# rskew/aiko_services

Measured on AMD Instinct MI355X. Metric: frames/sec (whole node) + p50 latency, ResNet-50 pipeline at 1/2/4/8 MI355X, higher is better.
Workload: dtype bf16; 1 GPU; global_batch=640, per_gpu_batch=640, parallelism=dp1, hipgraph=True, ingest=hbm, setup_frames=12, model=resnet50, pipeline=(SyntheticFrames ResNet50Classifier ClassifierTopK), gpu_lanes=2

## Files before the change

aiko_services_amd/csrc/kernels/conv_exp.hip:

```cpp
#include <type_traits>

#include "conv_common.h"
#include "conv_wide_stage.h"

namespace aiko {

typedef __attribute__((ext_vector_type(2))) short i16x2;

__device__ __forceinline__ uint32_t relu_bf16x2(uint32_t v) {
  return __builtin_bit_cast(uint32_t, __builtin_elementwise_max(__builtin_bit_cast(i16x2, v), i16x2{0, 0}));
}

struct ConvExpParams {
  ConvParams c;
  const bf16_t* w3;
  const float* b3;
  int N;
};

__global__ __launch_bounds__(512, 1) void conv3x3_exp_kernel(ConvExpParams q) {
  const ConvParams& p = q.c;
  constexpr int BM = 256, BN = 256, BK = 64, WGN = 4, NW = 8, NS = 2;
  constexpr int WM = 128, WN = 64, MI = 8, NI = 4, NP = 2;
  constexpr int RPW = 8, RPI = 64, APT = 4, BPT = 4;
  constexpr int STAGE_ELEMS = (BM + BN) * BK;
  constexpr int T2_BLOCK = BM * 64;
  static_assert(NS * STAGE_ELEMS == 4 * T2_BLOCK, "the t2 slice fills the ring exactly");
  __shared__ __attribute__((aligned(16))) bf16_t ring[NS * STAGE_ELEMS];

  const int wave = __builtin_amdgcn_readfirstlane(threadIdx.x >> 6);
  const int wr = wave / WGN, wc = wave % WGN;
  const int ntiles = (p.M + BM - 1) / BM;
  const int G = gridDim.x;
  const int lid = xcd_remap(blockIdx.x, G);

  const __amdgpu_buffer_rsrc_t rx = wide_rsrc(p.x);
  const __amdgpu_buffer_rsrc_t rw = wide_rsrc(p.w);
  const __amdgpu_buffer_rsrc_t rw3 = wide_rsrc(q.w3);
  const int io_bytes = p.M * q.N * 2;
  const __amdgpu_buffer_rsrc_t rr =
      __builtin_amdgcn_make_buffer_rsrc(const_cast<bf16_t*>(p.res), (short)0, io_bytes, 0x00020000);
  const __amdgpu_buffer_rsrc_t ry = __builtin_amdgcn_make_buffer_rsrc(p.y, (short)0, io_bytes, 0x00020000);

  const int nkb = p.K / BK;
  const int nch = q.N / 128;

  for (int tile = lid; tile < ntiles; tile += G) {
    const int m0 = tile * BM;
    uint32_t lz = 0u;
    asm volatile("" : "+v"(lz));
    const int lane1 = __builtin_amdgcn_mbcnt_hi(~0u, __builtin_amdgcn_mbcnt_lo(~0u, lz));
    const int lrow = wave * RPW + (lane1 >> 3);
    const int lp = (lane1 & 7) ^ (lane1 >> 3);
    const int HoWo = p.Ho * p.Wo;
    uint32_t b_off[BPT];
#pragma unroll
    for (int i = 0; i < BPT; ++i) b_off[i] = (uint32_t)(((lrow + RPI * i) * p.K + lp * 8) * 2);

    const int fr = lane1 & 15, fq = lane1 >> 4;
    const int coff = ((fq & 1) << 4) | ((fq >> 1) << 3);
    const int sw = fr & 7;

    int a_base[APT];
    uint32_t a_mask[APT], a_off[APT];
#pragma unroll
    for (int i = 0; i < APT; ++i) {
      const int m = m0 + lrow + RPI * i;
      a_mask[i] = 0u;
      a_base[i] = 0;
      a_off[i] = kWideOOB;
      if (m < p.M) {
        const int img = fdiv(m, p.mHoWo, p.lHoWo);
        const int rem = m - img * HoWo;
        const int oh = fdiv(rem, p.mWo, p.lWo);
        const int ow = rem - oh * p.Wo;
        const int ih0 = oh * p.stride - p.pad, iw0 = ow * p.stride - p.pad;
        a_base[i] = (((img * p.H + ih0) * p.W + iw0) * p.C + lp * 8) * 2;
        const int r_lo = max(0, -ih0), r_hi = min(p.R, p.H - ih0);
        const int s_lo = max(0, -iw0), s_hi = min(p.S, p.W - iw0);
        const uint32_t mr = r_hi > r_lo ? ((1u << r_hi) - 1u) & ~((1u << r_lo) - 1u) : 0u;
        const uint32_t ms = s_hi > s_lo ? ((1u << s_hi) - 1u) & ~((1u << s_lo) - 1u) : 0u;
        a_mask[i] = mr | (ms << 16);
      }
    }
    float e_bias[NP][8];
#pragma unroll
    for (int h = 0; h < NP; ++h) {
      const int n = wc * WN + h * 32 + coff;
      const f32x4 b0 = *reinterpret_cast<const f32x4*>(p.bias + n);
      const f32x4 b1 = *reinterpret_cast<const f32x4*>(p.bias + n + 4);
      e_bias[h][0] = b0[0]; e_bias[h][1] = b0[1]; e_bias[h][2] = b0[2]; e_bias[h][3] = b0[3];
      e_bias[h][4] = b1[0]; e_bias[h][5] = b1[1]; e_bias[h][6] = b1[2]; e_bias[h][7] = b1[3];
    }

    int cur_tap = -1, iss_tap = 0, iss_c = 0, iss_r = 0, iss_s = 0;
    auto issue = [&](int kb, auto slot_tag) {
      constexpr int SLOT = decltype(slot_tag)::value;
      bf16_t* Xs = ring + SLOT * STAGE_ELEMS;
      bf16_t* Ws = Xs + BM * BK;
      const uint32_t sb = (uint32_t)(kb * BK * 2);
#pragma unroll
      for (int i = 0; i < BPT; ++i) wide_dma16(rw, b_off[i], sb, Ws + (i * RPI + wave * RPW) * BK);
      if (iss_tap != cur_tap) {
        cur_tap = iss_tap;
        const int tap_off = ((iss_r * p.W + iss_s) * p.C) * 2;
        const uint32_t bit = (1u << iss_r) | (1u << (iss_s + 16));
#pragma unroll
        for (int i = 0; i < APT; ++i)
          a_off[i] = (a_mask[i] & bit) == bit ? (uint32_t)(a_base[i] + tap_off) : kWideOOB;
      }
      const uint32_t soff = (uint32_t)(iss_c * 2);
#pragma unroll
      for (int i = 0; i < APT; ++i) wide_dma16(rx, a_off[i], soff, Xs + (i * RPI + wave * RPW) * BK);
      iss_c += BK;
      if (iss_c >= p.Cc) {
        iss_c = 0;
        ++iss_tap;
        if (++iss_s == p.S) {
          iss_s = 0;
          ++iss_r;
        }
      }
    };

    f32x4 acc[NI][MI];
    float zero = 0.f;
    asm volatile("" : "+v"(zero));
#pragma unroll
    for (int j = 0; j < NI; ++j)
#pragma unroll
      for (int i = 0; i < MI; ++i) acc[j][i] = f32x4{zero, zero, zero, zero};

    int w_rd[NI], x_rd[MI];
#pragma unroll
    for (int j = 0; j < NI; ++j) w_rd[j] = BM * BK + (wc * WN + j * 16 + fr) * BK;
#pragma unroll
    for (int i = 0; i < MI; ++i) x_rd[i] = (wr * WM + i * 16 + fr) * BK;

    auto compute = [&](auto slot_tag) {
      constexpr int SLOT = decltype(slot_tag)::value;
      const bf16_t* St = ring + SLOT * STAGE_ELEMS;
#pragma unroll
      for (int kk = 0; kk < BK / 32; ++kk) {
        const int pc = ((fq + 4 * kk) ^ sw) << 3;
        bf16x8 wf[NI], xf[MI];
#pragma unroll
        for (int j = 0; j < NI; ++j) wf[j] = *reinterpret_cast<const bf16x8*>(St + w_rd[j] + pc);
#pragma unroll
        for (int i = 0; i < MI; ++i) xf[i] = *reinterpret_cast<const bf16x8*>(St + x_rd[i] + pc);
#pragma unroll
        for (int i = 0; i < MI; ++i)
#pragma unroll
          for (int j = 0; j < NI; ++j)
            acc[j][i] = __builtin_amdgcn_mfma_f32_16x16x32_bf16(wf[j], xf[i], acc[j][i], 0, 0, 0);
      }
    };

    auto step = [&](int kb, auto slot_tag) {
      constexpr int SLOT = decltype(slot_tag)::value;
      wide_vm_barrier<0>();
      if (kb + 1 < nkb) issue(kb + 1, std::integral_constant<int, 1 - SLOT>{});
      compute(slot_tag);
    };
    using S0 = std::integral_constant<int, 0>;
    using S1 = std::integral_constant<int, 1>;
    issue(0, S0{});
    {
      int kb = 0;
      for (; kb + 2 <= nkb; kb += 2) {
        step(kb, S0{});
        step(kb + 1, S1{});
      }
      if (kb < nkb) step(kb, S0{});
    }

    uint32_t lz2 = 0u;
    asm volatile("" : "+v"(lz2));
    const int lane2 = __builtin_amdgcn_mbcnt_hi(~0u, __builtin_amdgcn_mbcnt_lo(~0u, lz2));
    const int fr2 = lane2 & 15, fq2 = lane2 >> 4;
    const int coff2 = ((fq2 & 1) << 4) | ((fq2 >> 1) << 3);
    const int sw2 = fr2 & 7;
    const int x_r0 = (wr * WM + fr2) * 64;
    __syncthreads();
#pragma unroll
    for (int i = 0; i < MI; ++i) {
#pragma unroll
      for (int h = 0; h < NP; ++h) {
        f32x4 lo = acc[2 * h][i], hi = acc[2 * h + 1][i];
#pragma unroll
        for (int e = 0; e < 4; ++e) {
          const auto s = __builtin_amdgcn_permlane16_swap(__float_as_uint(lo[e]), __float_as_uint(hi[e]), false, false);
          lo[e] = __uint_as_float(s[0]);
          hi[e] = __uint_as_float(s[1]);
        }
        u32x4 o;
        o[0] = pack2(fmaxf(lo[0] + e_bias[h][0], 0.f), fmaxf(lo[1] + e_bias[h][1], 0.f));
        o[1] = pack2(fmaxf(lo[2] + e_bias[h][2], 0.f), fmaxf(lo[3] + e_bias[h][3], 0.f));
        o[2] = pack2(fmaxf(hi[0] + e_bias[h][4], 0.f), fmaxf(hi[1] + e_bias[h][5], 0.f));
        o[3] = pack2(fmaxf(hi[2] + e_bias[h][6], 0.f), fmaxf(hi[3] + e_bias[h][7], 0.f));
        const int piece = (h * 4 + (coff2 >> 3)) ^ sw2;
        *reinterpret_cast<u32x4*>(ring + wc * T2_BLOCK + (x_r0 + i * 16 * 64) + (piece << 3)) = o;
      }
    }

    const uint32_t row0 = (uint32_t)(((m0 + wr * WM + fr2) * q.N + wc * 32 + coff2) * 2);
    const uint32_t row_step = (uint32_t)(16 * q.N * 2);
    const uint32_t w_off = (uint32_t)(wc * 2 * 8 * 1024 + lane2 * 16);
    bf16x8 wreg[4][2];
    u32x4 e_res[2][MI];
    f32x2 e_b3[4];
    auto load_w = [&](int c, int ks) __attribute__((always_inline)) {
      const uint32_t base = c < nch ? w_off : kWideOOB;
#pragma unroll
      for (int j = 0; j < 2; ++j)
        wreg[ks & 3][j] = __builtin_bit_cast(bf16x8, __builtin_amdgcn_raw_buffer_load_b128(
            rw3, base, (uint32_t)c * 65536u + (uint32_t)((j * 8 + ks) * 1024), 0));
    };
    auto load_res = [&](int c, auto par_tag) __attribute__((always_inline)) {
      constexpr int P = decltype(par_tag)::value;
      const uint32_t cb = (uint32_t)c * 256u;
      const uint32_t base = c < nch ? row0 : kWideOOB;
      uint32_t rs = row_step;
      asm volatile("" : "+s"(rs));
#pragma unroll
      for (int i = 0; i < MI; ++i)
        e_res[P][i] = __builtin_bit_cast(u32x4, __builtin_amdgcn_raw_buffer_load_b128(
            rr, base + rs * i, cb, 0));
    };
    auto load_b3 = [&](int c) __attribute__((always_inline)) {
      const int n = c * 128 + wc * 32 + coff2;
      const f32x4 b0 = *reinterpret_cast<const f32x4*>(q.b3 + n);
      const f32x4 b1 = *reinterpret_cast<const f32x4*>(q.b3 + n + 4);
      e_b3[0] = f32x2{b0[0], b0[1]}; e_b3[1] = f32x2{b0[2], b0[3]};
      e_b3[2] = f32x2{b1[0], b1[1]}; e_b3[3] = f32x2{b1[2], b1[3]};
    };
    using P0 = std::integral_constant<int, 0>;
    using P1 = std::integral_constant<int, 1>;
#pragma unroll
    for (int ks = 0; ks < 4; ++ks) load_w(0, ks);
    load_res(0, P0{});
    load_res(1, P1{});
    __syncthreads();

    const bf16_t* xa[2][2];
#pragma unroll
    for (int par = 0; par < 2; ++par)
#pragma unroll
      for (int half = 0; half < 2; ++half)
        xa[par][half] = ring + half * 2 * T2_BLOCK + x_r0 + (((fq2 + 4 * par) ^ sw2) << 3);
    auto read_x = [&](int ks, int i) __attribute__((always_inline)) {
      return *reinterpret_cast<const bf16x8*>(xa[ks & 1][ks >> 2] + ((ks >> 1) & 1) * T2_BLOCK + i * 16 * 64);
    };
    bf16x8 xf[MI];
#pragma unroll
    for (int i = 0; i < MI; ++i) xf[i] = read_x(0, i);
    auto chunk = [&](int c, auto par_tag) __attribute__((always_inline)) {
      constexpr int P = decltype(par_tag)::value;
      asm volatile("" ::: "memory");
      f32x4 acc2[2][MI];
#pragma unroll
      for (int j = 0; j < 2; ++j)
#pragma unroll
        for (int i = 0; i < MI; ++i) acc2[j][i] = f32x4{0.f, 0.f, 0.f, 0.f};
      load_b3(c);
#pragma unroll
      for (int ks = 0; ks < 8; ++ks) {
#pragma unroll
        for (int i = 0; i < MI; ++i) {
#pragma unroll
          for (int j = 0; j < 2; ++j)
            acc2[j][i] = __builtin_amdgcn_mfma_f32_16x16x32_bf16(wreg[ks & 3][j], xf[i], acc2[j][i], 0, 0, 0);
          xf[i] = read_x((ks + 1) & 7, i);
          __builtin_amdgcn_sched_barrier(0);
        }
        if (ks < 4) load_w(c, ks + 4);
        else load_w(c + 1, ks - 4);
        __builtin_amdgcn_sched_barrier(0);
      }
      const uint32_t cb = (uint32_t)c * 256u;
      uint32_t rs = row_step;
      asm volatile("" : "+s"(rs));
#pragma unroll
      for (int i = 0; i < MI; ++i) {
        f32x4 lo = acc2[0][i], hi = acc2[1][i];
#pragma unroll
        for (int e = 0; e < 4; ++e) {
          const auto s = __builtin_amdgcn_permlane16_swap(__float_as_uint(lo[e]), __float_as_uint(hi[e]), false, false);
          lo[e] = __uint_as_float(s[0]);
          hi[e] = __uint_as_float(s[1]);
        }
        const f32x2 v[4] = {f32x2{lo[0], lo[1]} + e_b3[0], f32x2{lo[2], lo[3]} + e_b3[1],
                            f32x2{hi[0], hi[1]} + e_b3[2], f32x2{hi[2], hi[3]} + e_b3[3]};
        u32x4 o;
#pragma unroll
        for (int e = 0; e < 4; ++e) {
          const f32x2 r = {__uint_as_float(e_res[P][i][e] << 16), __uint_as_float(e_res[P][i][e] & 0xffff0000u)};
          const f32x2 t = v[e] + r;
          o[e] = relu_bf16x2(pack2(t[0], t[1]));
        }
        __builtin_amdgcn_raw_buffer_store_b128(o, ry, row0 + rs * i, cb, 0);
        asm volatile("s_nop 1");
        __builtin_amdgcn_sched_barrier(0);
      }
      load_res(c + 2, par_tag);
    };
    for (int c = 0; c < nch; c += 2) {
      chunk(c, P0{});
      chunk(c + 1, P1{});
    }
    __syncthreads();
  }
}

}

extern "C" int aiko_conv3x3_exp(const void* t1, const void* w2, const float* b2, const void* w3img,
                                const float* b3, const void* res, void* y, int B, int H, int W, int N,
                                int grid, hipStream_t stream) {
  using namespace aiko;
  const long M = (long)B * H * W;
  if (N <= 0 || N % 256 || M <= 0 || M * N * 2 >= 0x7ffffff0L || H * W <= 0 || grid < 0) return -1;
  ConvExpParams q;
  ConvParams& p = q.c;
  p.x = static_cast<const bf16_t*>(t1);
  p.w = static_cast<const bf16_t*>(w2);
  p.bias = b2;
  p.res = static_cast<const bf16_t*>(res);
  p.y = static_cast<bf16_t*>(y);
  p.H = H; p.W = W; p.C = 256; p.Cc = 256; p.R = 3; p.S = 3;
  p.stride = 1; p.pad = 1; p.Ho = H; p.Wo = W; p.M = (int)M; p.Cout = 256; p.K = 9 * 256;
  p.act = 1; p.ldy = N; p.ldr = N;
  p.x2 = nullptr;
  p.K1 = p.K; p.H2 = 0; p.W2 = 0; p.C2 = 0; p.stride2 = 1;
  conv_params_finalize(p);
  q.w3 = static_cast<const bf16_t*>(w3img);
  q.b3 = b3;
  q.N = N;
  const int ntiles = (int)((M + 255) / 256);
  const int g = grid > 0 && grid < ntiles ? grid : ntiles;
  conv3x3_exp_kernel<<<dim3(g), 512, 0, stream>>>(q);
  return (int)hipGetLastError();
}
```

Before: 100,000 frames/s.

## Stage expansion-conv weights through LDS with async DMA double buffering

Templates the fused 3x3+1x1 expansion kernel on a W3_LDS flag. When enabled (the default), the 1x1 weights for each chunk are DMA'd into two extra LDS slots ahead of use, with vmcnt waits and barriers between steps, instead of each wave loading them directly into registers. This aims to hide weight-load latency and cut redundant global traffic. In exchange it adds block-wide barriers per k-step and more LDS per block. An environment variable selects the old path.

```diff
diff --git a/aiko_services_amd/csrc/kernels/conv_exp.hip b/aiko_services_amd/csrc/kernels/conv_exp.hip
--- a/aiko_services_amd/csrc/kernels/conv_exp.hip
+++ b/aiko_services_amd/csrc/kernels/conv_exp.hip
@@ -1,3 +1,4 @@
+#include <cstdlib>
 #include <type_traits>
 
 #include "conv_common.h"
@@ -18,6 +19,7 @@
   int N;
 };
 
+template <bool W3_LDS>
 __global__ __launch_bounds__(512, 1) void conv3x3_exp_kernel(ConvExpParams q) {
   const ConvParams& p = q.c;
   constexpr int BM = 256, BN = 256, BK = 64, WGN = 4, NW = 8, NS = 2;
@@ -25,8 +27,10 @@
   constexpr int RPW = 8, RPI = 64, APT = 4, BPT = 4;
   constexpr int STAGE_ELEMS = (BM + BN) * BK;
   constexpr int T2_BLOCK = BM * 64;
+  constexpr int W3_SLOT = 128 * 64;
   static_assert(NS * STAGE_ELEMS == 4 * T2_BLOCK, "the t2 slice fills the ring exactly");
-  __shared__ __attribute__((aligned(16))) bf16_t ring[NS * STAGE_ELEMS];
+  static_assert((NS * STAGE_ELEMS + 2 * W3_SLOT) * 2 <= 160 * 1024, "LDS budget");
+  __shared__ __attribute__((aligned(16))) bf16_t ring[NS * STAGE_ELEMS + (W3_LDS ? 2 * W3_SLOT : 0)];
 
   const int wave = __builtin_amdgcn_readfirstlane(threadIdx.x >> 6);
   const int wr = wave / WGN, wc = wave % WGN;
@@ -181,7 +185,20 @@
     const int coff2 = ((fq2 & 1) << 4) | ((fq2 >> 1) << 3);
     const int sw2 = fr2 & 7;
     const int x_r0 = (wr * WM + fr2) * 64;
+    const int nst = nch * 4;
+    const uint32_t w_lane = (uint32_t)lane2 * 16u;
+    auto issue_w = [&](int g, int slot) __attribute__((always_inline)) {
+      bf16_t* dst = ring + NS * STAGE_ELEMS + slot * W3_SLOT + wave * 1024;
+      const uint32_t voff = g < nst ? w_lane : kWideOOB;
+      const uint32_t soff = (uint32_t)(g >> 2) * 65536u + (uint32_t)(wave * 8192 + (g & 3) * 2048);
+      wide_dma16(rw3, voff, soff, dst);
+      wide_dma16(rw3, voff, soff + 1024u, dst + 512);
+    };
     __syncthreads();
+    if constexpr (W3_LDS) {
+      issue_w(0, 0);
+      issue_w(1, 1);
+    }
 #pragma unroll
     for (int i = 0; i < MI; ++i) {
 #pragma unroll
@@ -236,11 +253,34 @@
     };
     using P0 = std::integral_constant<int, 0>;
     using P1 = std::integral_constant<int, 1>;
-#pragma unroll
-    for (int ks = 0; ks < 4; ++ks) load_w(0, ks);
-    load_res(0, P0{});
-    load_res(1, P1{});
-    __syncthreads();
+    auto epilogue = [&](int c, auto par_tag, f32x4 (&acc2)[2][MI]) __attribute__((always_inline)) {
+      constexpr int P = decltype(par_tag)::value;
+      const uint32_t cb = (uint32_t)c * 256u;
+      uint32_t rs = row_step;
+      asm volatile("" : "+s"(rs));
+#pragma unroll
+      for (int i = 0; i < MI; ++i) {
+        f32x4 lo = acc2[0][i], hi = acc2[1][i];
+#pragma unroll
+        for (int e = 0; e < 4; ++e) {
+          const auto s = __builtin_amdgcn_permlane16_swap(__float_as_uint(lo[e]), __float_as_uint(hi[e]), false, false);
+          lo[e] = __uint_as_float(s[0]);
+          hi[e] = __uint_as_float(s[1]);
+        }
+        const f32x2 v[4] = {f32x2{lo[0], lo[1]} + e_b3[0], f32x2{lo[2], lo[3]} + e_b3[1],
+                            f32x2{hi[0], hi[1]} + e_b3[2], f32x2{hi[2], hi[3]} + e_b3[3]};
+        u32x4 o;
+#pragma unroll
+        for (int e = 0; e < 4; ++e) {
+          const f32x2 r = {__uint_as_float(e_res[P][i][e] << 16), __uint_as_float(e_res[P][i][e] & 0xffff0000u)};
+          const f32x2 t = v[e] + r;
+          o[e] = relu_bf16x2(pack2(t[0], t[1]));
+        }
+        __builtin_amdgcn_raw_buffer_store_b128(o, ry, row0 + rs * i, cb, 0);
+        asm volatile("s_nop 1");
+        __builtin_amdgcn_sched_barrier(0);
+      }
+    };
 
     const bf16_t* xa[2][2];
 #pragma unroll
@@ -252,61 +292,104 @@
       return *reinterpret_cast<const bf16x8*>(xa[ks & 1][ks >> 2] + ((ks >> 1) & 1) * T2_BLOCK + i * 16 * 64);
     };
     bf16x8 xf[MI];
-#pragma unroll
-    for (int i = 0; i < MI; ++i) xf[i] = read_x(0, i);
-    auto chunk = [&](int c, auto par_tag) __attribute__((always_inline)) {
-      constexpr int P = decltype(par_tag)::value;
-      asm volatile("" ::: "memory");
-      f32x4 acc2[2][MI];
-#pragma unroll
-      for (int j = 0; j < 2; ++j)
-#pragma unroll
-        for (int i = 0; i < MI; ++i) acc2[j][i] = f32x4{0.f, 0.f, 0.f, 0.f};
-      load_b3(c);
-#pragma unroll
-      for (int ks = 0; ks < 8; ++ks) {
-#pragma unroll
-        for (int i = 0; i < MI; ++i) {
+    if constexpr (!W3_LDS) {
+#pragma unroll
+      for (int ks = 0; ks < 4; ++ks) load_w(0, ks);
+      load_res(0, P0{});
+      load_res(1, P1{});
+      __syncthreads();
+#pragma unroll
+      for (int i = 0; i < MI; ++i) xf[i] = read_x(0, i);
+      auto chunk = [&](int c, auto par_tag) __attribute__((always_inline)) {
+        asm volatile("" ::: "memory");
+        f32x4 acc2[2][MI];
+#pragma unroll
+        for (int j = 0; j < 2; ++j)
+#pragma unroll
+          for (int i = 0; i < MI; ++i) acc2[j][i] = f32x4{0.f, 0.f, 0.f, 0.f};
+        load_b3(c);
+#pragma unroll
+        for (int ks = 0; ks < 8; ++ks) {
+#pragma unroll
+          for (int i = 0; i < MI; ++i) {
+#pragma unroll
+            for (int j = 0; j < 2; ++j)
+              acc2[j][i] = __builtin_amdgcn_mfma_f32_16x16x32_bf16(wreg[ks & 3][j], xf[i], acc2[j][i], 0, 0, 0);
+            xf[i] = read_x((ks + 1) & 7, i);
+            __builtin_amdgcn_sched_barrier(0);
+          }
+          if (ks < 4) load_w(c, ks + 4);
+          else load_w(c + 1, ks - 4);
+          __builtin_amdgcn_sched_barrier(0);
+        }
+        epilogue(c, par_tag, acc2);
+        load_res(c + 2, par_tag);
+      };
+      for (int c = 0; c < nch; c += 2) {
+        chunk(c, P0{});
+        chunk(c + 1, P1{});
+      }
+    } else {
+      load_res(0, P0{});
+      wide_vm_barrier<10>();
+      const bf16_t* wrd = ring + NS * STAGE_ELEMS + wc * 2048 + lane2 * 8;
+      u32x4 wA[2][2], wB[2][2];
+      auto read_w = [&](auto slot_tag, u32x4 (&w)[2][2]) __attribute__((always_inline)) {
+        constexpr int SLOT = decltype(slot_tag)::value;
+#pragma unroll
+        for (int sl = 0; sl < 2; ++sl)
 #pragma unroll
           for (int j = 0; j < 2; ++j)
-            acc2[j][i] = __builtin_amdgcn_mfma_f32_16x16x32_bf16(wreg[ks & 3][j], xf[i], acc2[j][i], 0, 0, 0);
-          xf[i] = read_x((ks + 1) & 7, i);
-          __builtin_amdgcn_sched_barrier(0);
-        }
-        if (ks < 4) load_w(c, ks + 4);
-        else load_w(c + 1, ks - 4);
+            w[sl][j] = *reinterpret_cast<const u32x4*>(wrd + SLOT * W3_SLOT + j * 1024 + sl * 512);
+      };
+      auto step = [&](int c, auto kb_tag, auto par_tag, f32x4 (&acc2)[2][MI]) __attribute__((always_inline)) {
+        constexpr int KB = decltype(kb_tag)::value, CUR = KB & 1, P = decltype(par_tag)::value;
+        u32x4 (&wcur)[2][2] = CUR ? wB : wA;
+        u32x4 (&wnxt)[2][2] = CUR ? wA : wB;
+        asm volatile("s_waitcnt vmcnt(%4)\n\ts_barrier"
+                     : "+v"(wcur[0][0]), "+v"(wcur[0][1]), "+v"(wcur[1][0]), "+v"(wcur[1][1])
+                     : "n"(KB < 2 ? 8 : 0)
+                     : "memory");
+        issue_w(c * 4 + KB + 2, CUR);
+        if constexpr (KB == 0) {
+          load_b3(c);
+          load_res(c + 1, std::integral_constant<int, 1 - P>{});
+        }
+        read_w(std::integral_constant<int, 1 - CUR>{}, wnxt);
         __builtin_amdgcn_sched_barrier(0);
-      }
-      const uint32_t cb = (uint32_t)c * 256u;
-      uint32_t rs = row_step;
-      asm volatile("" : "+s"(rs));
-#pragma unroll
-      for (int i = 0; i < MI; ++i) {
-        f32x4 lo = acc2[0][i], hi = acc2[1][i];
-#pragma unroll
-        for (int e = 0; e < 4; ++e) {
-          const auto s = __builtin_amdgcn_permlane16_swap(__float_as_uint(lo[e]), __float_as_uint(hi[e]), false, false);
-          lo[e] = __uint_as_float(s[0]);
-          hi[e] = __uint_as_float(s[1]);
-        }
-        const f32x2 v[4] = {f32x2{lo[0], lo[1]} + e_b3[0], f32x2{lo[2], lo[3]} + e_b3[1],
-                            f32x2{hi[0], hi[1]} + e_b3[2], f32x2{hi[2], hi[3]} + e_b3[3]};
-        u32x4 o;
-#pragma unroll
-        for (int e = 0; e < 4; ++e) {
-          const f32x2 r = {__uint_as_float(e_res[P][i][e] << 16), __uint_as_float(e_res[P][i][e] & 0xffff0000u)};
-          const f32x2 t = v[e] + r;
-          o[e] = relu_bf16x2(pack2(t[0], t[1]));
-        }
-        __builtin_amdgcn_raw_buffer_store_b128(o, ry, row0 + rs * i, cb, 0);
-        asm volatile("s_nop 1");
-        __builtin_amdgcn_sched_barrier(0);
-      }
-      load_res(c + 2, par_tag);
-    };
-    for (int c = 0; c < nch; c += 2) {
-      chunk(c, P0{});
-      chunk(c + 1, P1{});
+#pragma unroll
+        for (int s2 = 0; s2 < 2; ++s2) {
+          constexpr int ks0 = 2 * KB;
+#pragma unroll
+          for (int i = 0; i < MI; ++i) {
+#pragma unroll
+            for (int j = 0; j < 2; ++j)
+              acc2[j][i] = __builtin_amdgcn_mfma_f32_16x16x32_bf16(__builtin_bit_cast(bf16x8, wcur[s2][j]), xf[i],
+                                                                  acc2[j][i], 0, 0, 0);
+            xf[i] = read_x((ks0 + s2 + 1) & 7, i);
+            __builtin_amdgcn_sched_barrier(0);
+          }
+        }
+      };
+      read_w(P0{}, wA);
+#pragma unroll
+      for (int i = 0; i < MI; ++i) xf[i] = read_x(0, i);
+      auto chunk = [&](int c, auto par_tag) __attribute__((always_inline)) {
+        f32x4 acc2[2][MI];
+#pragma unroll
+        for (int j = 0; j < 2; ++j)
+#pragma unroll
+          for (int i = 0; i < MI; ++i) acc2[j][i] = f32x4{0.f, 0.f, 0.f, 0.f};
+        step(c, std::integral_constant<int, 0>{}, par_tag, acc2);
+        step(c, std::integral_constant<int, 1>{}, par_tag, acc2);
+        step(c, std::integral_constant<int, 2>{}, par_tag, acc2);
+        step(c, std::integral_constant<int, 3>{}, par_tag, acc2);
+        epilogue(c, par_tag, acc2);
+      };
+      for (int c = 0; c < nch; c += 2) {
+        chunk(c, P0{});
+        chunk(c + 1, P1{});
+      }
     }
     __syncthreads();
   }
@@ -338,6 +421,10 @@
   q.N = N;
   const int ntiles = (int)((M + 255) / 256);
   const int g = grid > 0 && grid < ntiles ? grid : ntiles;
-  conv3x3_exp_kernel<<<dim3(g), 512, 0, stream>>>(q);
+  const char* w3 = getenv("AIKO_EXP_W3_LDS");
+  if (w3 && atoi(w3) == 0)
+    conv3x3_exp_kernel<false><<<dim3(g), 512, 0, stream>>>(q);
+  else
+    conv3x3_exp_kernel<true><<<dim3(g), 512, 0, stream>>>(q);
   return (int)hipGetLastError();
 }
```

Result: no change. 100,000 frames/s (median of 3 runs) (+0.0%).
